# ucas-vg/PointTinyBenchmark

Measured on AMD Instinct MI355X. Metric: img/s (640x640) CPR R50-FPN fwd+loss, higher is better.
Workload: dtype fp32

## Files before the change

### include/cpr_hip.h

```cpp
#ifndef CPR_HIP_H
#define CPR_HIP_H
#ifdef __cplusplus
extern "C" {
#endif

#define CPR_ERR_ARG (-1001)
#define CPR_ERR_UNSUPPORTED (-1002)

int cpr_version(void);

#define CPR_CONV_RELU 1
#define CPR_CONV_OUT_BF16 2
#define CPR_CONV_RES_MASK 4
#define CPR_CONV_COLSUM 8
int cpr_conv2d_fwd(const float* in, const float* wgt, float* out, const float* scale, const float* bias,
                   const float* residual, const float* in_a, const float* in_b, float* gn_part, int N, int H, int W,
                   int Cin, int Cout, int KH, int KW, int stride, int pad, int Kpad, int flags, int in_relu,
                   int* variant_out, void* stream);

int cpr_conv2d_dual_fwd(const float* in, const float* wgt, const float* in2, const float* wgt2, float* out,
                        const float* scale, const float* bias, const float* scale2, const float* bias2, int N, int H, int W,
                        int Cin, int Cout, int KH, int KW, int stride, int pad, int Kpad, int H2, int W2, int Cin2,
                        int stride2, int Kpad2, int flags, int* variant_out, void* stream);

int cpr_conv1x1_stream_fwd(const float* in, const float* wgt, float* out, const float* scale, const float* bias,
                           const float* residual, long long M, int Cin, int Cout, int flags, void* stream);

int cpr_conv_wgrad_bf16_workspace(int N, int H, int W, int Cin, int Cout, int k);
int cpr_conv_wgrad_bf16(const void* dy, int dy_bf16, const void* x, int x_bf16, float* grad, void* ws, int N, int H, int W, int Cin,
                        int Cout, int k, int accumulate, void* stream);
int cpr_wgrad_bf16_set_tn(int on);
int cpr_conv_wgrad_bf16_workspace_s(int N, int H, int W, int Cin, int Cout, int k, int stride);
int cpr_conv_wgrad_bf16_s(const void* dy, int dy_bf16, const void* x, int x_bf16, float* grad, void* ws, int N, int H, int W, int Cin,
                          int Cout, int k, int stride, int accumulate, void* stream);

#define CPR_WINO_IN_B8 1
#define CPR_WINO_OUT_B8 2
int cpr_wino_pack_weights(const float* wgt, float* u, int Cin, int Cout, int Kpad, void* stream);
int cpr_conv3x3_wino_fwd(const float* in, const float* u, float* out, const float* scale, const float* bias,
                         const float* in_a, const float* in_b, float* gn_part, int N, int H, int W, int Cin, int Cout,
                         int flags, int in_relu, int layout, void* stream);
int cpr_wino32_pack_weights(const float* wgt, float* u, int Cin, int Cout, int Kpad, void* stream);
int cpr_conv3x3_wino32_slots(int H, int W);
int cpr_conv3x3_wino32_fwd(const float* in, const float* u, float* out, const float* scale, const float* bias,
                           const float* in_a, const float* in_b, float* gn_part, int N, int H, int W, int Cin, int Cout,
                           int flags, int in_relu, int layout, void* stream);
int cpr_gn_apply_b8(const float* x, const float* a, const float* b, float* y, int N, int H, int W, int C, int relu,
                    void* stream);

int cpr_conv2d_fwd_bf16(const void* in, const void* wgt, const void* wgt_frag, void* out, const float* scale, const float* bias,
                        const void* residual, float* gn_part, int N, int H, int W, int Cin, int Cout, int KH, int KW,
                        int stride, int pad, int Kpad, int relu, int out_fp32, int* variant_out, void* stream);
int cpr_conv2d_bf16_mask_slots(int N, int H, int W, int Cin, int Cout, int KH, int KW, int stride, int pad, int out_fp32);
int cpr_conv2d_dgrad_bf16_fused(const void* in, const void* wgt, const void* wgt_frag, float* out32, void* out16, const float* add32,
                                const void* mask, float* part, int N, int H, int W, int Cin, int Cout, int KH, int KW, int stride,
                                int pad, int Kpad, int* variant_out, void* stream);
int cpr_stem7x7s2_bf16(const float* in, const void* wgt, const float* scale, const float* bias, void* out, int N, int H, int W,
                       int relu, int layout, void* stream);
int cpr_stem7x7s2_pool_bf16(const float* in, const void* wgt, const float* scale, const float* bias, void* out, int N, int H,
                            int W, int layout, void* stream);
int cpr_maxpool3x3s2_bf16(const void* in, void* out, int N, int H, int W, int C, void* stream);
int cpr_gn_stats_bf16(const void* x, float* part, int N, int HW, int C, int P, void* stream);
int cpr_gn_apply_bf16(const void* x, const float* a, const float* b, const void* up, void* y, int N, int H, int W,
                      int C, int UH, int UW, int relu, void* stream);

int cpr_nchw_to_nhwc4(const float* in, float* out, int N, int C, int H, int W, void* stream);
int cpr_nhwc_to_nchw(const float* in, float* out, int N, int C, int H, int W, void* stream);
int cpr_stem7x7s2_pool_f32(const float* in, const float* wgt, const float* scale, const float* bias, float* out, int N, int H,
                           int W, int layout, void* stream);
// ... 177 lines not shown
int cpr_sgd_step(float* p, const float* grad, float* buf, const double* norm2, long long n, float lr, float mu, float wd,
                 float max_norm, float grad_scale, int first, void* stream);
int cpr_adam_step(float* p, const float* grad, float* exp_avg, float* exp_avg_sq, const double* norm2, long long n, double lr,
                  double beta1, double beta2, double eps, double wd, float step_size, float bc2_sqrt, float max_norm,
                  float grad_scale, int decoupled, void* stream);

int cpr_preprocess_u8(const unsigned char* img, const int* flip, const float* mean3, const float* stdinv3, int to_rgb,
                      float* out, int N, int H, int W, int Hp, int Wp, void* stream);
int cpr_clip_flip_boxes(float* boxes, const int* img_of, const int* flip, const int* img_hw, int n, int clip,
                        void* stream);

#ifdef CPR_BENCH_HOOKS
int cpr_conv_force_tile(int bm, int bn);
int cpr_conv_set_pipeline(int mode);
int cpr_conv_set_stream(int on);
int cpr_conv_set_ablation(int mode);
int cpr_wgrad_set_ablation(int mode);
int cpr_conv_set_extra_lds(int bytes);
int cpr_wino_set_variant(int sched, int ablate);
int cpr_bf16_set_dma(int on);
int cpr_bf16_set_wfrag(int on);
int cpr_wino_set_staging(int var, int tpx);
int cpr_wino32_set_debug(int ablate, int wg_per_cu, int stagger_pct);
int cpr_lsa_phase_clocks(long long* host_out, int reset);
#endif

#ifdef __cplusplus
}
#endif
#endif
```

### pointtinybenchmark_amd/_lib.py

```python
import ctypes
import os

_HERE = os.path.dirname(os.path.abspath(__file__))
LIB_PATH = os.path.join(_HERE, 'csrc', 'libcprhip.so')

_p = ctypes.c_void_p
_i = ctypes.c_int
_f = ctypes.c_float
_l = ctypes.c_longlong
_d = ctypes.c_double

SIGNATURES = {
    'cpr_version': [],
    'cpr_conv2d_fwd': [_p, _p, _p, _p, _p, _p, _p, _p, _p, _i, _i, _i, _i, _i, _i, _i, _i, _i, _i, _i, _i, _p, _p],
    'cpr_conv2d_dual_fwd': [_p] * 9 + [_i] * 16 + [_p, _p],
    'cpr_conv1x1_stream_fwd': [_p, _p, _p, _p, _p, _p, _l, _i, _i, _i, _p],
    'cpr_conv_wgrad_bf16_workspace': [_i, _i, _i, _i, _i, _i],
    'cpr_conv_wgrad_bf16_workspace_s': [_i] * 7,
    'cpr_conv_wgrad_bf16': [_p, _i, _p, _i, _p, _p, _i, _i, _i, _i, _i, _i, _i, _p],
    'cpr_conv_wgrad_bf16_s': [_p, _i, _p, _i, _p, _p] + [_i] * 8 + [_p],
    'cpr_wino_pack_weights': [_p, _p, _i, _i, _i, _p],
    'cpr_conv3x3_wino_fwd': [_p, _p, _p, _p, _p, _p, _p, _p, _i, _i, _i, _i, _i, _i, _i, _i, _p],
    'cpr_wino32_pack_weights': [_p, _p, _i, _i, _i, _p],
    'cpr_conv3x3_wino32_slots': [_i, _i],
    'cpr_conv3x3_wino32_fwd': [_p, _p, _p, _p, _p, _p, _p, _p, _i, _i, _i, _i, _i, _i, _i, _i, _p],
    'cpr_conv3x3_wino_wgrad_workspace': [_i, _i, _i, _i, _i],
    'cpr_conv3x3_wino_wgrad': [_p, _p, _p, _p, _p, _p, _i, _i, _i, _i, _i, _i, _i, _p],
    'cpr_gn_apply_b8': [_p, _p, _p, _p, _i, _i, _i, _i, _i, _p],
    'cpr_conv2d_fwd_bf16': [_p, _p, _p, _p, _p, _p, _p, _p] + [_i] * 12 + [_p, _p],
    'cpr_conv2d_bf16_mask_slots': [_i] * 10,
    'cpr_wgrad_bf16_set_tn': [_i],
    'cpr_bn_fold_multi': [_p, _i, _i, _p],
    'cpr_pack_weights_multi': [_p, _i, _i, _p],
    'cpr_pack_weights_bf16_multi': [_p, _i, _i, _p],
    'cpr_conv2d_dgrad_bf16_fused': [_p] * 8 + [_i] * 10 + [_p, _p],
    'cpr_stem7x7s2_bf16': [_p, _p, _p, _p, _p, _i, _i, _i, _i, _i, _p],
    'cpr_stem7x7s2_pool_bf16': [_p, _p, _p, _p, _p, _i, _i, _i, _i, _p],
    'cpr_maxpool3x3s2_bf16': [_p, _p, _i, _i, _i, _i, _p],
    'cpr_gn_stats_bf16': [_p, _p, _i, _i, _i, _i, _p],
    'cpr_gn_apply_bf16': [_p, _p, _p, _p, _p, _i, _i, _i, _i, _i, _i, _i, _p],
    'cpr_nchw_to_nhwc4': [_p, _p, _i, _i, _i, _i, _p],
    'cpr_nhwc_to_nchw': [_p, _p, _i, _i, _i, _i, _p],
    'cpr_stem7x7s2_pool_f32': [_p, _p, _p, _p, _p, _i, _i, _i, _i, _p],
    'cpr_maxpool3x3s2': [_p, _p, _i, _i, _i, _i, _p],
    'cpr_maxpool3x3s2_rec': [_p, _p, _p, _i, _i, _i, _i, _p],
    'cpr_maxpool3x3s2_bf16_rec': [_p, _p, _p, _i, _i, _i, _i, _p],
# ... 58 lines not shown
    'cpr_bn_apply': [_p] * 10 + [_l, _i, _i, _p],
    'cpr_bn_train_bwd': [_p] * 11 + [_l, _i, _p],
    'cpr_p2p_out_bf16_fwd': [_p] * 7 + [_i] * 5 + [_p],
    'cpr_p2p_out_bf16_dgrad': [_p, _i, _p, _p] + [_i] * 6 + [_p],
    'cpr_p2p_out_bf16_wgrad_ws': [_i] * 5,
    'cpr_p2p_out_bf16_wgrad': [_p] * 4 + [_i] + [_p] * 3 + [_i] * 5 + [_p],
    'cpr_p2p_loss_bwd': [_p] * 9 + [_i] * 5 + [_f] * 9 + [_p, _i, _i, _p],
    'cpr_p2p_loss_bwd_levels': [_p] * 7 + [_i] * 5 + [_p] * 6 + [_f] * 9 + [_p, _i, _i, _p],
    'cpr_grad_sumsq': [_p, _l, _p, _p, _i, _p],
    'cpr_sgd_step': [_p, _p, _p, _p, _l, _f, _f, _f, _f, _f, _i, _p],
    'cpr_adam_step': [_p, _p, _p, _p, _p, _l, _d, _d, _d, _d, _d, _f, _f, _f, _f, _i, _p],
}

BENCH_SIGNATURES = {
    'cpr_lsa_phase_clocks': [_p, _i],
    'cpr_wino32_set_debug': [_i, _i, _i],
    'cpr_conv_force_tile': [_i, _i],
    'cpr_conv_set_pipeline': [_i],
    'cpr_conv_set_stream': [_i],
    'cpr_conv_set_ablation': [_i],
    'cpr_wgrad_set_ablation': [_i],
    'cpr_wino_set_variant': [_i, _i],
    'cpr_wino_set_staging': [_i, _i],
    'cpr_conv_set_extra_lds': [_i],
    'cpr_bf16_set_dma': [_i],
    'cpr_bf16_set_wfrag': [_i],
}
BENCH_LIB_PATH = os.path.join(_HERE, 'csrc', 'libcprhip_bench.so')

_lib = None


class CprHipError(RuntimeError):
    pass


def load():
    global _lib
    if _lib is not None:
        return _lib
    path, sigs = LIB_PATH, dict(SIGNATURES)
    if os.environ.get('CPR_BENCH_HOOKS', '0') == '1':
        path = BENCH_LIB_PATH
        sigs.update(BENCH_SIGNATURES)
    if not os.path.exists(path):
        raise CprHipError('%s not found: run `python -m pointtinybenchmark_amd.build%s` (no CPU fallback exists)'
# ... 24 lines not shown
```

### pointtinybenchmark_amd/build.py

```python
import os
import subprocess
import sys

CSRC = os.path.join(os.path.dirname(os.path.abspath(__file__)), 'csrc')
LIB = os.path.join(CSRC, 'libcprhip.so')
SOURCES = ['conv_mfma.hip', 'conv1x1_stream.hip', 'conv_mfma_bf16.hip', 'conv_bf16_dma.hip', 'conv_bf16_pp.hip', 'stem_bf16.hip', 'stem_f32.hip', 'conv_wgrad_bf16.hip', 'conv_wgrad_bf16_tn.hip', 'conv_wgrad.hip', 'norm_pool.hip', 'cpr_points.hip', 'assign.hip',
           'postproc.hip', 'backward.hip', 'preprocess.hip', 'pack.hip', 'project.hip', 'conv_wino.hip', 'conv_wino32.hip', 'conv_wino_wgrad.hip', 'bn_train.hip',
           'p2p_out_bf16.hip', 'optim.hip', 'stem_bwd.hip']
HEADERS = ['common.h', 'conv_bf16_dma.h']
EXACT_SOURCES = {'cpr_points.hip', 'assign.hip', 'postproc.hip', 'preprocess.hip', 'optim.hip'}


def _hipcc():
    for c in (os.environ.get('HIPCC'), '/opt/rocm/bin/hipcc', 'hipcc'):
        if c and (os.path.isabs(c) and os.path.exists(c) or not os.path.isabs(c)):
            return c
    return 'hipcc'


def needs_build():
    if not os.path.exists(LIB):
        return True
    t = os.path.getmtime(LIB)
    deps = [os.path.join(CSRC, s) for s in SOURCES + HEADERS]
    return any(os.path.getmtime(d) > t for d in deps if os.path.exists(d))


BENCH_LIB = os.path.join(CSRC, 'libcprhip_bench.so')
HOOK_SOURCES = {'conv_mfma.hip', 'conv_wgrad.hip', 'conv_wino.hip', 'conv_mfma_bf16.hip', 'conv_bf16_dma.hip', 'conv_bf16_pp.hip', 'assign.hip', 'conv_wino32.hip'}


def build(force=False, verbose=True, bench_hooks=False):
    lib = BENCH_LIB if bench_hooks else LIB
    if not force and not (needs_build() if not bench_hooks else (
            not os.path.exists(lib) or any(os.path.getmtime(os.path.join(CSRC, s)) > os.path.getmtime(lib)
                                           for s in SOURCES + HEADERS))):
        return lib
    objs = []
    for s in SOURCES:
        src = os.path.join(CSRC, s)
        if not os.path.exists(src):
            continue
        hooked = bench_hooks and s in HOOK_SOURCES
        obj = os.path.join(CSRC, s.replace('.hip', '.bench.o' if hooked else '.o'))
        if bench_hooks and not hooked and os.path.exists(obj) and os.path.getmtime(obj) >= os.path.getmtime(src) \
                and all(os.path.getmtime(obj) >= os.path.getmtime(os.path.join(CSRC, h)) for h in HEADERS):
            objs.append(obj)
            continue
        cmd = [_hipcc(), '--offload-arch=gfx950', '-O3', '-std=c++17', '-fPIC'] + \
            (['-ffp-contract=off'] if s in EXACT_SOURCES else []) + (['-DCPR_BENCH_HOOKS'] if hooked else []) + \
            ['-c', src, '-o', obj]
        if verbose:
# ... 15 lines not shown
```

### pointtinybenchmark_amd/layers.py

```python
import os
import struct

import torch
import torch.nn as nn

from . import _lib, ops


_WEIGHT_EPOCH = [0]


def bump_weight_epoch():
    _WEIGHT_EPOCH[0] += 1


REFRESH_IN_PLACE = [os.environ.get('CPR_REFRESH_IN_PLACE', '1') != '0']

_FOLDS, _PACKS16, _PACKS32 = 'cpr_bn_fold_multi', 'cpr_pack_weights_bf16_multi', 'cpr_pack_weights_multi'


class FoldJob:
    multi = _FOLDS
    fold = None
    _ROW = struct.Struct('<7Qif')
# ... 13 lines not shown
    _ROW16, _ROW32 = struct.Struct('<4Q8i'), struct.Struct('<3Q10i')

    def __init__(self, weight, value, transpose, fold):
        self.weight, self.value, self.transpose, self.fold = weight, value, transpose, fold
        self.shape = O, I, KH, KW = weight.shape
        rows, cols = (I, O) if transpose else (O, I)
        bf16 = value.dtype == torch.bfloat16
        self.multi = _PACKS16 if bf16 else _PACKS32
        self.nblocks = max(1, min(64, (rows * (KH * KW * cols // 2 if bf16 else value.Kpad) + 255) // 256))

    def ptrs(self):
        pc = self.value
        return (self.weight.data_ptr(), 0 if self.fold is None else self.fold.value[0].data_ptr(), pc.w.data_ptr(),
                0 if pc.wfrag is None else pc.wfrag.data_ptr())

    def row(self, ptrs, block0):
        pc, nb = self.value, self.nblocks
        if self.multi is _PACKS16:
            return self._ROW16.pack(*ptrs, *self.shape, self.transpose, block0, nb, 0), block0 + nb
        return self._ROW32.pack(*ptrs[:3], nb, 0, *self.shape, pc.Cin, pc.Kpad, self.transpose, block0), block0 + nb

    def refresh_images(self, stream):
        pc = self.value
        for img, fn in ((pc.wino, 'cpr_wino_pack_weights'), (pc.wino32, 'cpr_wino32_pack_weights')):
            if img is not None:
                _lib.call(fn, pc.w.data_ptr(), img.data_ptr(), pc.Cin, pc.Cout, pc.Kpad, stream)


def _pack_job(pc, weight, transpose=0, fold=None):
    if isinstance(pc, ops.PackedConv) and weight.is_cuda and weight.dtype == torch.float32 and weight.is_contiguous() and \
            (pc.dtype == torch.float32 or ops.PACK_BF16_KERNEL[0]):
        return PackJob(weight, pc, transpose, fold)
    return None


class _Entry:
    __slots__ = ('tensors', 'ver', 'val', 'ready')

    def __init__(self, tensors, ver, val, ready):
        self.tensors, self.ver, self.val, self.ready = tensors, ver, val, ready


class _PackCache:

    def __init__(self):
        self._d = {}
        self._jobs = {}
# ... 177 lines not shown
```

### pointtinybenchmark_amd/ops.py

```python
import collections
import ctypes
import math
import os

import torch

from . import _lib


def _ptr(t):
    return ctypes.c_void_p(t.data_ptr()) if t is not None else None


def _stream():
    return ctypes.c_void_p(torch.cuda.current_stream().cuda_stream)


def _check(t, dtype=torch.float32):
    if not t.is_cuda:
        raise _lib.CprHipError('HIP op called with a CPU tensor: the product path has no CPU fallback')
    ok = t.dtype in dtype if isinstance(dtype, tuple) else t.dtype == dtype
    assert ok and t.is_contiguous(), (t.dtype, t.stride())
    return t

# ... 13 lines not shown


def nchw_to_nhwc(x):
    N, C, H, W = x.shape
    if C <= 4:
        x = _check(x.contiguous())
        out = torch.empty((N, H, W, 4), device=x.device, dtype=torch.float32)
        _lib.call('cpr_nchw_to_nhwc4', _ptr(x), _ptr(out), N, C, H, W, _stream())
        return out
    return x.permute(0, 2, 3, 1).contiguous()


def nhwc_to_nchw_dense(x_nhwc):
    N, H, W, C = x_nhwc.shape
    out = torch.empty((N, C, H, W), device=x_nhwc.device, dtype=torch.float32)
    _lib.call('cpr_nhwc_to_nchw', _ptr(_check(x_nhwc)), _ptr(out), N, C, H, W, _stream())
    return out


class PackedConv:
    wfrag = None
    wino = None
    wino32 = None
    ready = None

    def _packed(self):
        self.ready = record_ready()

    def __init__(self, weight, stride=1, padding=0, dtype=torch.float32):
        Cout, Cin, KH, KW = weight.shape
        w = weight.detach().to(torch.float32).permute(0, 2, 3, 1)
        self.dtype = dtype
        if dtype == torch.bfloat16:
            assert Cin % 64 == 0, 'bf16 conv needs Cin % 64 == 0'
            self.Cout, self.Cin, self.KH, self.KW, self.Kpad = Cout, Cin, KH, KW, KH * KW * Cin
            self.stride, self.padding = stride, padding
            if weight.is_cuda and PACK_BF16_KERNEL[0]:
                self._pack_bf16(weight, None, 0)
                return
            self.w = w.reshape(Cout, KH * KW * Cin).to(torch.bfloat16).contiguous()
            return
        if Cin <= 4:
            cin_p = 4
        else:
            assert Cin % 32 == 0, 'input channels must be a multiple of 32 (or <= 4 for the stem)'
            cin_p = Cin
# ... 100 lines not shown
    cur = torch.cuda.current_stream()
    if cur.cuda_stream != stream:
        cur.wait_event(ev)
    return ready


def pack_ready(pc):
    if pc.ready is not None:
        pc.ready = wait_ready(pc.ready)


def wino_eligible(pc, H, W, dtype=torch.float32):
    if not (WINOGRAD[0] and dtype == torch.float32 and pc.dtype == torch.float32 and pc.KH == 3 and pc.KW == 3 and
            pc.stride == 1 and pc.padding == 1 and pc.Cin % 16 == 0 and pc.Cin >= 32 and pc.Cout % 64 == 0):
        return False
    fill = (H * W) / float(((H + 15) // 16 * 16) * ((W + 15) // 16 * 16))
    return fill >= WINO_MIN_FILL


WINO_TILE = [os.environ.get('CPR_WINO_TILE', 'auto')]


def wino_instance(pc, H, W, fused_affine):
    can32 = pc.Cin % 8 == 0 and (not fused_affine or pc.Cin <= 256)
    if WINO_TILE[0] == '64' or not can32:
        return '64'
    if WINO_TILE[0] == '32':
        return '32'
    return WINO_AUTO(pc, H, W, fused_affine)


WINO32_MAX_PIXELS = 40 * 40


def WINO_AUTO(pc, H, W, fused_affine):
    return '32' if H * W <= WINO32_MAX_PIXELS else '64'


def wino_gn_slots(pc, H, W, fused_affine):
    if wino_instance(pc, H, W, fused_affine) == '32':
        return ((H + 7) // 8) * ((W + 15) // 16)
    return ((H + 15) // 16) * ((W + 15) // 16)


def is_b8(x):
    return x.dim() == 5 and x.shape[-1] == 8


def conv3x3_wino(x, pc, scale=None, bias=None, relu=False, gn_part=False, out=None, in_ab=None, in_relu=False,
                 out_b8=False):
    _check(x, ACT)
    in_b8 = is_b8(x)
    if in_b8:
        N, _, H, W, _ = x.shape
        Cin = x.shape[1] * 8
    else:
        N, H, W, Cin = x.shape
    assert x.dtype == torch.float32 and Cin == pc.Cin and pc.KH == 3 and pc.stride == 1 and pc.padding == 1
    inst = wino_instance(pc, H, W, in_ab is not None)
    attr, pack_fn = ('wino32', 'cpr_wino32_pack_weights') if inst == '32' else ('wino', 'cpr_wino_pack_weights')
    if getattr(pc, attr) is None:
        pack_ready(pc)
        wino = torch.empty((16 * pc.Cin * pc.Cout,), device=x.device, dtype=torch.float32)
        _lib.call(pack_fn, _ptr(pc.w), _ptr(wino), pc.Cin, pc.Cout, pc.Kpad, _stream())
        setattr(pc, attr, wino)
        pc._packed()
    pack_ready(pc)
    shape = (N, pc.Cout // 8, H, W, 8) if out_b8 else (N, H, W, pc.Cout)
    if out is None:
        out = torch.empty(shape, device=x.device, dtype=torch.float32)
    assert tuple(out.shape) == shape and out.is_contiguous()
    part = None
    if gn_part:
        part = torch.empty((N * wino_gn_slots(pc, H, W, in_ab is not None), pc.Cout, 2), device=x.device, dtype=torch.float32)
    a = b = None
    if in_ab is not None:
        a, b = in_ab
        assert Cin <= 512
    _lib.call('cpr_conv3x3_wino32_fwd' if inst == '32' else 'cpr_conv3x3_wino_fwd', _ptr(x), _ptr(getattr(pc, attr)), _ptr(out),
              _ptr(scale), _ptr(bias), _ptr(a), _ptr(b), _ptr(part), N, H, W, Cin, pc.Cout, CONV_RELU if relu else 0, int(in_relu),
              (1 if in_b8 else 0) | (2 if out_b8 else 0), _stream())
    if TRACE_CONV_VARIANT[0]:
        TRACE_CONV_VARIANT[1] = ('wino32' if inst == '32' else 'wino',
                                 (1 if in_b8 else 0) | (2 if out_b8 else 0) | (4 if in_ab is not None else 0))
    return (out, part) if gn_part else out


def gn_apply_b8(x, a=None, b=None, relu=False):
    assert is_b8(x)
    N, C8, H, W, _ = _check(x, ACT).shape
    y = torch.empty((N, H, W, C8 * 8), device=x.device, dtype=torch.float32)
    _lib.call('cpr_gn_apply_b8', _ptr(x), _ptr(a), _ptr(b), _ptr(y), N, H, W, C8 * 8, int(relu), _stream())
    return y


def conv2d(x, pc, scale=None, bias=None, residual=None, relu=False, in_ab=None, in_relu=False, gn_part=False,
           out=None, out_dtype=None, res_mask=False, colsum=False, out_b8=False):
    _check(x, ACT)
    pack_ready(pc)
    if is_b8(x):
        assert residual is None and not (res_mask or colsum) and out_dtype in (None, torch.float32) and \
            wino_eligible(pc, x.shape[2], x.shape[3], x.dtype), 'channel-blocked input needs a Winograd-eligible layer'
        return conv3x3_wino(x, pc, scale, bias, relu, gn_part, out, in_ab, in_relu, out_b8)
    N, H, W, Cin = x.shape
    assert Cin == pc.Cin, (Cin, pc.Cin)
    assert x.dtype == pc.dtype, 'weights were packed for %s, input is %s' % (pc.dtype, x.dtype)
    OH, OW = pc.out_hw(H, W)
# ... 1112 lines not shown
```

Baseline: 905.8.

## Add bf16 three-way-split Winograd 3x3 conv kernel for large wide layers

Adds a new Winograd F(2x2,3x3) forward kernel that splits fp32 transformed inputs and weights into three bf16 pieces (high, mid, low) and accumulates products with bf16 MFMA instructions, emulating fp32 accuracy. The auto-selector now routes 3x3 layers with at least 256 input and output channels and at least 160x160 pixels to this kernel, with a matching weight-packing path and weight-refresh hook. The aim is to replace slower fp32 matrix throughput with the higher bf16 MFMA rate on the largest FPN and head convolutions. The cost is several extra MFMAs per product, triple-size weight images, and a small residual precision difference from exact fp32.

```diff
diff --git a/include/cpr_hip.h b/include/cpr_hip.h
--- a/include/cpr_hip.h
+++ b/include/cpr_hip.h
@@ -45,6 +45,10 @@
 int cpr_conv3x3_wino32_fwd(const float* in, const float* u, float* out, const float* scale, const float* bias,
                            const float* in_a, const float* in_b, float* gn_part, int N, int H, int W, int Cin, int Cout,
                            int flags, int in_relu, int layout, void* stream);
+int cpr_wino_split_pack_weights(const float* wgt, void* u, int Cin, int Cout, int Kpad, void* stream);
+int cpr_conv3x3_wino_split_fwd(const float* in, const void* u, float* out, const float* scale, const float* bias,
+                               const float* in_a, const float* in_b, float* gn_part, int N, int H, int W, int Cin, int Cout,
+                               int flags, int in_relu, int layout, void* stream);
 int cpr_gn_apply_b8(const float* x, const float* a, const float* b, float* y, int N, int H, int W, int C, int relu,
                     void* stream);
 
@@ -268,6 +272,7 @@
 int cpr_bf16_set_wfrag(int on);
 int cpr_wino_set_staging(int var, int tpx);
 int cpr_wino32_set_debug(int ablate, int wg_per_cu, int stagger_pct);
+int cpr_wino_split_set_debug(int tpx, int scalar);
 int cpr_lsa_phase_clocks(long long* host_out, int reset);
 #endif
 
diff --git a/pointtinybenchmark_amd/_lib.py b/pointtinybenchmark_amd/_lib.py
--- a/pointtinybenchmark_amd/_lib.py
+++ b/pointtinybenchmark_amd/_lib.py
@@ -22,6 +22,8 @@
     'cpr_wino_pack_weights': [_p, _p, _i, _i, _i, _p],
     'cpr_conv3x3_wino_fwd': [_p, _p, _p, _p, _p, _p, _p, _p, _i, _i, _i, _i, _i, _i, _i, _i, _p],
     'cpr_wino32_pack_weights': [_p, _p, _i, _i, _i, _p],
+    'cpr_wino_split_pack_weights': [_p, _p, _i, _i, _i, _p],
+    'cpr_conv3x3_wino_split_fwd': [_p, _p, _p, _p, _p, _p, _p, _p, _i, _i, _i, _i, _i, _i, _i, _i, _p],
     'cpr_conv3x3_wino32_slots': [_i, _i],
     'cpr_conv3x3_wino32_fwd': [_p, _p, _p, _p, _p, _p, _p, _p, _i, _i, _i, _i, _i, _i, _i, _i, _p],
     'cpr_conv3x3_wino_wgrad_workspace': [_i, _i, _i, _i, _i],
@@ -126,6 +128,7 @@
     'cpr_wgrad_set_ablation': [_i],
     'cpr_wino_set_variant': [_i, _i],
     'cpr_wino_set_staging': [_i, _i],
+    'cpr_wino_split_set_debug': [_i, _i],
     'cpr_conv_set_extra_lds': [_i],
     'cpr_bf16_set_dma': [_i],
     'cpr_bf16_set_wfrag': [_i],
diff --git a/pointtinybenchmark_amd/build.py b/pointtinybenchmark_amd/build.py
--- a/pointtinybenchmark_amd/build.py
+++ b/pointtinybenchmark_amd/build.py
@@ -5,7 +5,7 @@
 CSRC = os.path.join(os.path.dirname(os.path.abspath(__file__)), 'csrc')
 LIB = os.path.join(CSRC, 'libcprhip.so')
 SOURCES = ['conv_mfma.hip', 'conv1x1_stream.hip', 'conv_mfma_bf16.hip', 'conv_bf16_dma.hip', 'conv_bf16_pp.hip', 'stem_bf16.hip', 'stem_f32.hip', 'conv_wgrad_bf16.hip', 'conv_wgrad_bf16_tn.hip', 'conv_wgrad.hip', 'norm_pool.hip', 'cpr_points.hip', 'assign.hip',
-           'postproc.hip', 'backward.hip', 'preprocess.hip', 'pack.hip', 'project.hip', 'conv_wino.hip', 'conv_wino32.hip', 'conv_wino_wgrad.hip', 'bn_train.hip',
+           'postproc.hip', 'backward.hip', 'preprocess.hip', 'pack.hip', 'project.hip', 'conv_wino.hip', 'conv_wino32.hip', 'conv_wino_split.hip', 'conv_wino_wgrad.hip', 'bn_train.hip',
            'p2p_out_bf16.hip', 'optim.hip', 'stem_bwd.hip']
 HEADERS = ['common.h', 'conv_bf16_dma.h']
 EXACT_SOURCES = {'cpr_points.hip', 'assign.hip', 'postproc.hip', 'preprocess.hip', 'optim.hip'}
@@ -27,7 +27,7 @@
 
 
 BENCH_LIB = os.path.join(CSRC, 'libcprhip_bench.so')
-HOOK_SOURCES = {'conv_mfma.hip', 'conv_wgrad.hip', 'conv_wino.hip', 'conv_mfma_bf16.hip', 'conv_bf16_dma.hip', 'conv_bf16_pp.hip', 'assign.hip', 'conv_wino32.hip'}
+HOOK_SOURCES = {'conv_mfma.hip', 'conv_wgrad.hip', 'conv_wino.hip', 'conv_mfma_bf16.hip', 'conv_bf16_dma.hip', 'conv_bf16_pp.hip', 'assign.hip', 'conv_wino32.hip', 'conv_wino_split.hip'}
 
 
 def build(force=False, verbose=True, bench_hooks=False):
diff --git a/pointtinybenchmark_amd/csrc/conv_wino_split.hip b/pointtinybenchmark_amd/csrc/conv_wino_split.hip
--- /dev/null
+++ b/pointtinybenchmark_amd/csrc/conv_wino_split.hip
@@ -0,0 +1,533 @@
+#include "common.h"
+
+typedef __bf16 bf16x8 __attribute__((ext_vector_type(8)));
+typedef __bf16 bf16x4 __attribute__((ext_vector_type(4)));
+typedef __bf16 bf16x2 __attribute__((ext_vector_type(2)));
+typedef float f32x2 __attribute__((ext_vector_type(2)));
+typedef unsigned u32x4 __attribute__((ext_vector_type(4)));
+
+struct WinoSplitParams {
+    const float* in;
+    const __bf16* u;
+    float* out;
+    const float* scale;
+    const float* bias;
+    float* gn_part;
+    const float* in_a;
+    const float* in_b;
+    int in_relu, out_b8;
+    int N, H, W, Cin, Cout, relu, RY, RX, regions, tilesN, nch;
+    int tpx;
+};
+
+constexpr int SPLIT_UCHUNK = 16 * 2 * 3 * 256;
+constexpr int SPLIT_VBUF = 3 * 16 * 64 * 8;
+
+__device__ __forceinline__ void split3(f32x2 x, bf16x2& h, bf16x2& m, bf16x2& l) {
+    h = __builtin_convertvector(x, bf16x2);
+    const f32x2 r = x - __builtin_convertvector(h, f32x2);
+    m = __builtin_convertvector(r, bf16x2);
+    const f32x2 s = r - __builtin_convertvector(m, f32x2);
+    l = __builtin_convertvector(s, bf16x2);
+}
+
+__device__ __forceinline__ float sadd(float a, float b) { float r; asm("v_add_f32 %0, %1, %2" : "=v"(r) : "v"(a), "v"(b)); return r; }
+__device__ __forceinline__ float ssub(float a, float b) { float r; asm("v_sub_f32 %0, %1, %2" : "=v"(r) : "v"(a), "v"(b)); return r; }
+__device__ __forceinline__ float sfma(float a, float b, float c) {
+    float r; asm("v_fma_f32 %0, %1, %2, %3" : "=v"(r) : "v"(a), "v"(b), "v"(c)); return r;
+}
+__device__ __forceinline__ void split3s(float x0, float x1, bf16x2& h, bf16x2& m, bf16x2& l) {
+    h = __builtin_convertvector(f32x2{x0, x1}, bf16x2);
+    const float r0 = ssub(x0, (float)h[0]), r1 = ssub(x1, (float)h[1]);
+    m = __builtin_convertvector(f32x2{r0, r1}, bf16x2);
+    l = __builtin_convertvector(f32x2{ssub(r0, (float)m[0]), ssub(r1, (float)m[1])}, bf16x2);
+}
+
+__global__ void wino_split_pack_kernel(const float* __restrict__ w, __bf16* __restrict__ u, int Cin, int Cout, int Kpad) {
+    const int idx = blockIdx.x * blockDim.x + threadIdx.x;
+    if (idx >= Cin * Cout) return;
+    const int ci = idx % Cin, co = idx / Cin;
+    float g[3][3];
+#pragma unroll
+    for (int a = 0; a < 3; ++a)
+#pragma unroll
+        for (int b = 0; b < 3; ++b) g[a][b] = w[(size_t)co * Kpad + (a * 3 + b) * Cin + ci];
+    float t[4][3];
+#pragma unroll
+    for (int b = 0; b < 3; ++b) {
+        t[0][b] = g[0][b];
+        t[1][b] = 0.5f * (g[0][b] + g[1][b] + g[2][b]);
+        t[2][b] = 0.5f * (g[0][b] - g[1][b] + g[2][b]);
+        t[3][b] = g[2][b];
+    }
+    const int tn = co >> 6, cl = co & 63, chunk = ci >> 3, k = ci & 7, nch = Cin >> 3;
+    __bf16* dst = u + (size_t)(tn * nch + chunk) * SPLIT_UCHUNK + (cl >> 5) * 3 * 256 + (cl & 31) * 8 + k;
+#pragma unroll
+    for (int i = 0; i < 4; ++i) {
+        const float v[4] = {t[i][0], 0.5f * (t[i][0] + t[i][1] + t[i][2]), 0.5f * (t[i][0] - t[i][1] + t[i][2]), t[i][2]};
+#pragma unroll
+        for (int j = 0; j < 4; j += 2) {
+            bf16x2 h, m, l;
+            split3(f32x2{v[j], v[j + 1]}, h, m, l);
+#pragma unroll
+            for (int e = 0; e < 2; ++e) {
+                __bf16* d = dst + (i * 4 + j + e) * (2 * 3 * 256);
+                d[0] = h[e]; d[256] = m[e]; d[512] = l[e];
+            }
+        }
+    }
+}
+
+template <bool INB8, bool XF, bool SC>
+__global__ __launch_bounds__(512, 1) void conv_wino_split_kernel(WinoSplitParams p) {
+    constexpr int XFMAX = 512;
+    constexpr int RAWROW = 148;
+    constexpr int RAWBUF = 18 * RAWROW;
+    constexpr int VFLOATS = SPLIT_VBUF;
+    constexpr int KLOOP = VFLOATS + 2 * RAWBUF;
+    constexpr int EPI = 8 * 64 * 64;
+    constexpr int BASE = KLOOP > EPI ? KLOOP : EPI;
+    __shared__ __attribute__((aligned(16))) float smem[BASE + (XF ? 4 * XFMAX : 0)];
+    __bf16* Vs = reinterpret_cast<__bf16*>(smem);
+    float* Rw = smem + VFLOATS;
+    float* ABs = smem + BASE;
+
+    const int tid = threadIdx.x, lane = tid & 63;
+    const int wave = __builtin_amdgcn_readfirstlane(tid >> 6);
+    const int l31 = lane & 31, half = lane >> 5;
+
+    const int pixbytes = INB8 ? 32 : p.Cin * 4;
+    const int chunk_bytes = INB8 ? p.H * p.W * 32 : 32;
+    const __amdgpu_buffer_rsrc_t rs_in = __builtin_amdgcn_make_buffer_rsrc(
+        const_cast<float*>(p.in), 0, (int)((size_t)p.N * p.H * p.W * p.Cin * 4), 0x00020000);
+    const __amdgpu_buffer_rsrc_t rs_u = __builtin_amdgcn_make_buffer_rsrc(
+        const_cast<__bf16*>(p.u), 0, (int)((size_t)p.tilesN * p.nch * SPLIT_UCHUNK * 2), 0x00020000);
+    int par = 0;
+    int upyx[2], raw_wr[2];
+#pragma unroll
+    for (int k = 0; k < 2; ++k) {
+        const int pix = (tid + 512 * k) >> 1;
+        const int py = pix / 18, px = pix - py * 18;
+        upyx[k] = py << 8 | px;
+        raw_wr[k] = py * RAWROW + px * 8 + (tid & 1) * 4;
+    }
+    const bool second_unit = wave < 3;
+    const bool unit1_live = tid + 512 < 648;
+    const int ti = wave >> 1, ttl = (tid >> 1) & 63, tch = tid & 1;
+    const int t_ra = ti == 0 ? 0 : ti == 2 ? 2 : 1;
+    const int t_rb = ti == 0 ? 2 : ti == 1 ? 2 : ti == 2 ? 1 : 3;
+    const float t_sg = ti == 1 ? 1.f : -1.f;
+    const float* t_rd = Rw + (2 * (ttl & 7)) * RAWROW + (2 * (ttl >> 3)) * 8 + 4 * tch;
+    __bf16* const t_wr = Vs + (ti * 4) * 512 + ttl * 8 + 4 * tch;
+    const int last = p.nch - 1;
+    const float relu_floor = (XF && p.in_relu) ? 0.f : -INFINITY;
+
+    struct Tile {
+        int rg, tn, n, oy0, ox0, n0;
+        int voffA[2];
+        unsigned uok;
+        bool any_pad, valid;
+    };
+    const int T = p.regions * p.tilesN;
+    const int per = (T + 7) >> 3;
+    const int ngrp = p.tpx > 0 ? p.tilesN / p.tpx : 1;
+    const int per_r = p.tpx > 0 ? (p.regions * ngrp + 7) / 8 : 0;
+    auto setup = [&](int vb) {
+        Tile t;
+        if (p.tpx > 0) {
+            const int x = vb & 7, s = vb >> 3;
+            const int sr = s / p.tpx;
+            t.rg = (x / ngrp) * per_r + sr;
+            t.tn = (x % ngrp) * p.tpx + (s - sr * p.tpx);
+            t.valid = sr < per_r && t.rg < p.regions;
+            if (!t.valid) { t.rg = 0; t.tn = 0; }
+        } else {
+            const int tile = (vb & 7) * per + (vb >> 3);
+            t.valid = vb < per * 8 && tile < T;
+            const int tl = t.valid ? tile : 0;
+            t.rg = tl / p.tilesN; t.tn = tl - t.rg * p.tilesN;
+        }
+        t.n = t.rg / (p.RY * p.RX);
+        const int rrem = t.rg - t.n * p.RY * p.RX;
+        const int ry = rrem / p.RX, rx = rrem - ry * p.RX;
+        t.oy0 = ry * 16; t.ox0 = rx * 16; t.n0 = t.tn * 64;
+        const int img_base = INB8 ? (t.n * (p.Cin >> 3)) * p.H * p.W * 32 : t.n * p.H * p.W * p.Cin * 4;
+        t.uok = 0;
+#pragma unroll
+        for (int k = 0; k < 2; ++k) {
+            const int iy = t.oy0 - 1 + (upyx[k] >> 8), ix = t.ox0 - 1 + (upyx[k] & 255);
+            const bool ok = (k == 0 || unit1_live) & ((unsigned)iy < (unsigned)p.H) & ((unsigned)ix < (unsigned)p.W);
+            t.uok |= (ok ? 1u : 0u) << k;
+            t.voffA[k] = ok ? img_base + (iy * p.W + ix) * pixbytes + (tid & 1) * 16 : (int)0x80000000;
+        }
+        t.any_pad = XF && __builtin_amdgcn_ballot_w64(t.uok != (unit1_live ? 3u : 1u)) != 0;
+        return t;
+    };
+
+    f32x4 sp[2][2];
+    bf16x8 bx[2][2], by[2][2];
+    float tab_a = 0.f, tab_b = 0.f;
+    Tile cur = setup(blockIdx.x);
+    auto ld_a = [&](const Tile& t, int ck, int k) {
+        return __builtin_bit_cast(f32x4, __builtin_amdgcn_raw_buffer_load_b128(rs_in, t.voffA[k], ck * chunk_bytes, 0));
+    };
+    const int ub_x = (half ? 1 : 0) * 512 + l31 * 16, ub_y = (half ? 2 : 0) * 512 + l31 * 16;
+    auto ld_u = [&](int tn, int ck, int fl, int nb) {
+        const int f = 2 * wave + fl;
+        const int soff = (tn * p.nch + ck) * (SPLIT_UCHUNK * 2) + (f * 2 + nb) * 3 * 512;
+        bx[fl][nb] = __builtin_bit_cast(bf16x8, __builtin_amdgcn_raw_buffer_load_b128(rs_u, ub_x, soff, 0));
+        by[fl][nb] = __builtin_bit_cast(bf16x8, __builtin_amdgcn_raw_buffer_load_b128(rs_u, ub_y, soff, 0));
+    };
+    auto prefetch = [&](const Tile& t) {
+        sp[0][0] = ld_a(t, 0, 0); sp[1][0] = ld_a(t, 1, 0);
+        if (second_unit) { sp[0][1] = ld_a(t, 0, 1); sp[1][1] = ld_a(t, 1, 1); }
+#pragma unroll
+        for (int fl = 0; fl < 2; ++fl)
+#pragma unroll
+            for (int nb = 0; nb < 2; ++nb) ld_u(t.tn, 0, fl, nb);
+        if (XF) {
+            if (tid < p.Cin) { tab_a = p.in_a[t.n * p.Cin + tid]; tab_b = p.in_b[t.n * p.Cin + tid]; }
+        }
+    };
+    auto affine = [&](f32x4 v, f32x4 a4, f32x4 b4, int k) {
+        if (SC) v = f32x4{sfma(v.x, a4.x, b4.x), sfma(v.y, a4.y, b4.y), sfma(v.z, a4.z, b4.z), sfma(v.w, a4.w, b4.w)};
+        else v = v * a4 + b4;
+        v.x = fmaxf(v.x, relu_floor); v.y = fmaxf(v.y, relu_floor); v.z = fmaxf(v.z, relu_floor); v.w = fmaxf(v.w, relu_floor);
+        if (cur.any_pad) {
+            asm volatile("");
+            if (!((cur.uok >> k) & 1u)) v = f32x4{0.f, 0.f, 0.f, 0.f};
+        }
+        return v;
+    };
+    auto r_a = [&](f32x4 v, int chunk, int buf, int k) {
+        if (k == 1 && !second_unit) return;
+        if (XF) {
+            const float* tab = ABs + par * 2 * XFMAX + (chunk < last ? chunk : last) * 8 + (tid & 1) * 4;
+            v = affine(v, *reinterpret_cast<const f32x4*>(tab), *reinterpret_cast<const f32x4*>(tab + XFMAX), k);
+        }
+        if (k == 0 || unit1_live) *reinterpret_cast<f32x4*>(Rw + buf * RAWBUF + raw_wr[k]) = v;
+    };
+    f32x4 tr[4], ta[4];
+    auto t_read = [&](int buf, int s0) {
+#pragma unroll
+        for (int s = 0; s < 2; ++s) {
+            ta[2 * s] = *reinterpret_cast<const f32x4*>(t_rd + buf * RAWBUF + t_ra * RAWROW + (s0 + s) * 8);
+            ta[2 * s + 1] = *reinterpret_cast<const f32x4*>(t_rd + buf * RAWBUF + t_rb * RAWROW + (s0 + s) * 8);
+        }
+    };
+    auto t_pass = [&](int s0) {
+#pragma unroll
+        for (int s = 0; s < 2; ++s) {
+            const f32x4 a = ta[2 * s], b = ta[2 * s + 1];
+            if (SC) tr[s0 + s] = f32x4{sfma(t_sg, b.x, a.x), sfma(t_sg, b.y, a.y), sfma(t_sg, b.z, a.z), sfma(t_sg, b.w, a.w)};
+            else tr[s0 + s] = a + t_sg * b;
+        }
+    };
+    auto t_col = [&](int buf, int j) {
+        bf16x2 h0, m0, l0, h1, m1, l1;
+        if (SC) {
+            const f32x4 a = j == 0 ? tr[0] : j == 1 ? tr[1] : j == 2 ? tr[2] : tr[1];
+            const f32x4 b = j == 0 ? tr[2] : j == 1 ? tr[2] : j == 2 ? tr[1] : tr[3];
+            float o[4];
+#pragma unroll
+            for (int e = 0; e < 4; ++e) o[e] = j == 1 ? sadd(a[e], b[e]) : ssub(a[e], b[e]);
+            split3s(o[0], o[1], h0, m0, l0);
+            split3s(o[2], o[3], h1, m1, l1);
+        } else {
+            const f32x4 o = j == 0 ? tr[0] - tr[2] : j == 1 ? tr[1] + tr[2] : j == 2 ? tr[2] - tr[1] : tr[1] - tr[3];
+            split3(f32x2{o.x, o.y}, h0, m0, l0);
+            split3(f32x2{o.z, o.w}, h1, m1, l1);
+        }
+        __bf16* d = t_wr + buf * SPLIT_VBUF + j * 512;
+        *reinterpret_cast<bf16x4*>(d) = bf16x4{h0.x, h0.y, h1.x, h1.y};
+        *reinterpret_cast<bf16x4*>(d + 16 * 512) = bf16x4{m0.x, m0.y, m1.x, m1.y};
+        *reinterpret_cast<bf16x4*>(d + 32 * 512) = bf16x4{l0.x, l0.y, l1.x, l1.y};
+    };
+    const __bf16* a_lds = Vs + (2 * wave) * 512 + l31 * 8;
+    const int a3_plane = half ? 0 : 2;
+    bf16x8 fa[3];
+    auto a_read = [&](int buf, int fl, int tb, int z) {
+        const __bf16* b0 = a_lds + buf * SPLIT_VBUF + fl * 512 + tb * 256;
+        fa[z] = *reinterpret_cast<const bf16x8*>(b0 + (z == 0 ? 0 : z == 1 ? 16 * 512 : a3_plane * 16 * 512));
+    };
+
+    if (cur.valid) prefetch(cur);
+    if (XF) {
+        if (tid < p.Cin) { ABs[tid] = tab_a; ABs[XFMAX + tid] = tab_b; }
+        __syncthreads();
+    }
+    for (int vb = blockIdx.x; cur.valid; vb += gridDim.x) {
+    const int rg = cur.rg, n = cur.n, oy0 = cur.oy0, ox0 = cur.ox0, n0 = cur.n0;
+
+    f32x16 acc[2][2][2];
+#pragma unroll
+    for (int fl = 0; fl < 2; ++fl)
+#pragma unroll
+        for (int tb = 0; tb < 2; ++tb)
+#pragma unroll
+            for (int nb = 0; nb < 2; ++nb)
+#pragma unroll
+                for (int r = 0; r < 16; ++r) acc[fl][tb][nb][r] = 0.f;
+
+    r_a(sp[0][0], 0, 0, 0); r_a(sp[0][1], 0, 0, 1);
+    r_a(sp[1][0], 1, 1, 0); r_a(sp[1][1], 1, 1, 1);
+    sp[0][0] = ld_a(cur, 2 < last ? 2 : last, 0);
+    if (second_unit) sp[0][1] = ld_a(cur, 2 < last ? 2 : last, 1);
+    __syncthreads();
+    t_read(0, 0); t_pass(0); t_read(0, 2); t_pass(2);
+#pragma unroll
+    for (int j = 0; j < 4; ++j) t_col(0, j);
+    __syncthreads();
+#pragma unroll
+    for (int z = 0; z < 3; ++z) a_read(0, 0, 0, z);
+
+#define SMFMA(FL, TB)                                                                                            \
+    do {                                                                                                         \
+        acc[FL][TB][0] = __builtin_amdgcn_mfma_f32_32x32x16_bf16(fa[0], bx[FL][0], acc[FL][TB][0], 0, 0, 0);   \
+        q_fill(q++);                                                                                             \
+        acc[FL][TB][1] = __builtin_amdgcn_mfma_f32_32x32x16_bf16(fa[0], bx[FL][1], acc[FL][TB][1], 0, 0, 0);   \
+        q_fill(q++);                                                                                             \
+        acc[FL][TB][0] = __builtin_amdgcn_mfma_f32_32x32x16_bf16(fa[1], bx[FL][0], acc[FL][TB][0], 0, 0, 0);   \
+        q_fill(q++);                                                                                             \
+        acc[FL][TB][1] = __builtin_amdgcn_mfma_f32_32x32x16_bf16(fa[1], bx[FL][1], acc[FL][TB][1], 0, 0, 0);   \
+        q_fill(q++);                                                                                             \
+        acc[FL][TB][0] = __builtin_amdgcn_mfma_f32_32x32x16_bf16(fa[2], by[FL][0], acc[FL][TB][0], 0, 0, 0);   \
+        q_fill(q++);                                                                                             \
+        acc[FL][TB][1] = __builtin_amdgcn_mfma_f32_32x32x16_bf16(fa[2], by[FL][1], acc[FL][TB][1], 0, 0, 0);   \
+        q_fill(q++);                                                                                             \
+    } while (0)
+    for (int c = 0; c < p.nch; ++c) {
+        const int buf = c & 1, nbuf = buf ^ 1;
+        const int cn = c + 1 < last ? c + 1 : last;
+        auto q_fill = [&](int q) {
+            if (q & 1) {
+                const int g = q / 6 + 1, z = (q % 6) >> 1;
+                if (g < 4) a_read(buf, g >> 1, g & 1, z);
+                else a_read(nbuf, 0, 0, z);
+            }
+            switch (q) {
+                case 0: t_read(nbuf, 0); break;
+                case 2: t_pass(0); t_read(nbuf, 2); break;
+                case 3: t_pass(2); break;
+                case 4: t_col(nbuf, 0); break;
+                case 6: t_col(nbuf, 1); break;
+                case 8: t_col(nbuf, 2); break;
+                case 10: t_col(nbuf, 3); break;
+                case 12: ld_u(cur.tn, cn, 0, 0); ld_u(cur.tn, cn, 0, 1); break;
+                case 13: r_a(sp[0][0], c + 2, buf, 0); break;
+                case 14: r_a(sp[0][1], c + 2, buf, 1); break;
+                case 17:
+                    asm volatile("" ::: "memory");
+                    __builtin_amdgcn_s_waitcnt(0xc07f);
+                    __builtin_amdgcn_s_barrier();
+                    asm volatile("" ::: "memory");
+                    break;
+                case 18: {
+                    const int c3 = c + 3 < last ? c + 3 : last;
+                    sp[0][0] = ld_a(cur, c3, 0);
+                    if (second_unit) sp[0][1] = ld_a(cur, c3, 1);
+                    break;
+                }
+                case 23: ld_u(cur.tn, cn, 1, 0); ld_u(cur.tn, cn, 1, 1); break;
+                default: break;
+            }
+            __builtin_amdgcn_sched_barrier(0);
+        };
+        int q = 0;
+        SMFMA(0, 0);
+        SMFMA(0, 1);
+        SMFMA(1, 0);
+        SMFMA(1, 1);
+    }
+#undef SMFMA
+
+    const Tile nxt = setup(vb + gridDim.x);
+    if (nxt.valid) prefetch(nxt);
+    __syncthreads();
+    float* Rs = smem;
+    const int ei = wave >> 1, ejp = wave & 1;
+    if (ejp) {
+#pragma unroll
+        for (int tb = 0; tb < 2; ++tb)
+#pragma unroll
+            for (int nb = 0; nb < 2; ++nb)
+#pragma unroll
+                for (int r = 0; r < 16; ++r) {
+                    const int trow = tb * 32 + (r & 3) + 8 * (r >> 2) + 4 * half;
+                    const float m2 = acc[0][tb][nb][r], m3 = acc[1][tb][nb][r];
+                    Rs[((ei * 2 + 0) * 64 + trow) * 64 + nb * 32 + l31] = m2;
+                    Rs[((ei * 2 + 1) * 64 + trow) * 64 + nb * 32 + l31] = -m2 - m3;
+                }
+    }
+    __syncthreads();
+    if (!ejp) {
+#pragma unroll
+        for (int tb = 0; tb < 2; ++tb)
+#pragma unroll
+            for (int nb = 0; nb < 2; ++nb)
+#pragma unroll
+                for (int r = 0; r < 16; ++r) {
+                    const int trow = tb * 32 + (r & 3) + 8 * (r >> 2) + 4 * half;
+                    const float m0 = acc[0][tb][nb][r], m1 = acc[1][tb][nb][r];
+                    float* r0 = Rs + ((ei * 2 + 0) * 64 + trow) * 64 + nb * 32 + l31;
+                    float* r1 = Rs + ((ei * 2 + 1) * 64 + trow) * 64 + nb * 32 + l31;
+                    *r0 = (m0 + m1) + *r0;
+                    *r1 = m1 + *r1;
+                }
+    }
+    __syncthreads();
+    const int c4 = tid & 15;
+    const int co = n0 + c4 * 4;
+    f32x4 sc = {1.f, 1.f, 1.f, 1.f}, bi = {0.f, 0.f, 0.f, 0.f};
+    if (p.scale) sc = *reinterpret_cast<const f32x4*>(p.scale + co);
+    if (p.bias) bi = *reinterpret_cast<const f32x4*>(p.bias + co);
+    const __amdgpu_buffer_rsrc_t rs_out = __builtin_amdgcn_make_buffer_rsrc(
+        p.out, 0, (int)((size_t)p.N * p.H * p.W * p.Cout * 4), 0x00020000);
+    f32x4 gs = {0.f, 0.f, 0.f, 0.f}, gq = {0.f, 0.f, 0.f, 0.f};
+#pragma unroll
+    for (int k = 0; k < 2; ++k) {
+        const int t = (tid >> 4) + 32 * k;
+        const int oy = oy0 + 2 * (t & 7), ox = ox0 + 2 * (t >> 3);
+#pragma unroll
+        for (int b = 0; b < 2; ++b) {
+            const f32x4 r0 = *reinterpret_cast<const f32x4*>(Rs + ((0 * 2 + b) * 64 + t) * 64 + c4 * 4);
+            const f32x4 r1 = *reinterpret_cast<const f32x4*>(Rs + ((1 * 2 + b) * 64 + t) * 64 + c4 * 4);
+            const f32x4 r2 = *reinterpret_cast<const f32x4*>(Rs + ((2 * 2 + b) * 64 + t) * 64 + c4 * 4);
+            const f32x4 r3 = *reinterpret_cast<const f32x4*>(Rs + ((3 * 2 + b) * 64 + t) * 64 + c4 * 4);
+            f32x4 y[2] = {r0 + r1 + r2, r1 - r2 - r3};
+#pragma unroll
+            for (int a = 0; a < 2; ++a) {
+                f32x4 v = y[a] * sc + bi;
+                if (p.relu) { v.x = fmaxf(v.x, 0.f); v.y = fmaxf(v.y, 0.f); v.z = fmaxf(v.z, 0.f); v.w = fmaxf(v.w, 0.f); }
+                const bool ok = (oy + a < p.H) & (ox + b < p.W);
+                const unsigned off = !ok ? 0x80000000u
+                    : p.out_b8 ? (unsigned)((((n * (p.Cout >> 3) + (co >> 3)) * p.H + oy + a) * p.W + ox + b) * 8 + (co & 7)) * 4u
+                               : (unsigned)(((n * p.H + oy + a) * p.W + ox + b) * p.Cout + co) * 4u;
+                __builtin_amdgcn_raw_buffer_store_b128(__builtin_bit_cast(u32x4, v), rs_out, (int)off, 0, 0);
+                if (p.gn_part && ok) { gs += v; gq += v * v; }
+            }
+        }
+    }
+    if (p.gn_part) {
+#pragma unroll
+        for (int e = 0; e < 4; ++e) {
+            gs[e] += __shfl_xor(gs[e], 16, 64); gs[e] += __shfl_xor(gs[e], 32, 64);
+            gq[e] += __shfl_xor(gq[e], 16, 64); gq[e] += __shfl_xor(gq[e], 32, 64);
+        }
+        __syncthreads();
+        if (lane < 16) {
+#pragma unroll
+            for (int e = 0; e < 4; ++e) {
+                smem[(wave * 64 + c4 * 4 + e) * 2 + 0] = gs[e];
+                smem[(wave * 64 + c4 * 4 + e) * 2 + 1] = gq[e];
+            }
+        }
+        __syncthreads();
+        if (tid < 64) {
+            float s = 0.f, q = 0.f;
+#pragma unroll
+            for (int w8 = 0; w8 < 8; ++w8) { s += smem[(w8 * 64 + tid) * 2]; q += smem[(w8 * 64 + tid) * 2 + 1]; }
+            float* dst = p.gn_part + ((size_t)rg * p.Cout + n0 + tid) * 2;
+            dst[0] = s; dst[1] = q;
+        }
+    }
+    if (XF && tid < p.Cin) {
+        ABs[(par ^ 1) * 2 * XFMAX + tid] = tab_a;
+        ABs[(par ^ 1) * 2 * XFMAX + XFMAX + tid] = tab_b;
+    }
+    par ^= 1;
+    __syncthreads();
+    cur = nxt;
+    }
+}
+
+#ifdef CPR_BENCH_HOOKS
+static int split_tpx = -1, split_scalar = -1;
+extern "C" int cpr_wino_split_set_debug(int tpx, int scalar) {
+    CPR_CHECK_ARG(tpx >= -1 && tpx <= 2 && scalar >= -1 && scalar <= 1);
+    split_tpx = tpx;
+    split_scalar = scalar;
+    return CPR_OK;
+}
+#else
+constexpr int split_tpx = -1, split_scalar = -1;
+#endif
+constexpr int SPLIT_TPX_DEFAULT = 0, SPLIT_SCALAR_DEFAULT = 0;
+
+extern "C" int cpr_wino_split_pack_weights(const float* wgt, void* u, int Cin, int Cout, int Kpad, hipStream_t stream) {
+    CPR_CHECK_ARG(wgt && u && Cin > 0 && Cout > 0 && Cin % 8 == 0 && Cout % 64 == 0 && Kpad >= 9 * Cin);
+    hipLaunchKernelGGL(wino_split_pack_kernel, dim3(cdiv(Cin * Cout, 256)), dim3(256), 0, stream, wgt,
+                       static_cast<__bf16*>(u), Cin, Cout, Kpad);
+    CPR_LAUNCH_STATUS();
+}
+
+static int wino_split_launch(const float* in, const void* u, float* out, const float* scale, const float* bias,
+                             const float* in_a, const float* in_b, float* gn_part, int N, int H, int W, int Cin,
+                             int Cout, int flags, int in_relu, int layout, hipStream_t stream) {
+    CPR_CHECK_ARG(in && u && out && N > 0 && H > 0 && W > 0);
+    CPR_CHECK_ARG(Cin > 0 && Cout > 0 && Cin % 16 == 0 && Cout % 64 == 0 && Cin >= 32);
+    CPR_CHECK_ARG((flags & ~CPR_CONV_RELU) == 0 && (layout & ~3) == 0);
+    if (in_a) CPR_CHECK_ARG(in_b && Cin <= 512);
+    if ((long long)N * H * W * Cin * 4 >= (1ll << 31) || (long long)N * H * W * Cout * 4 >= (1ll << 31)) return CPR_ERR_UNSUPPORTED;
+    if ((long long)Cin * Cout * 96 >= (1ll << 31)) return CPR_ERR_UNSUPPORTED;
+    WinoSplitParams p;
+    p.in = in; p.u = static_cast<const __bf16*>(u); p.out = out; p.scale = scale; p.bias = bias; p.gn_part = gn_part;
+    p.in_a = in_a; p.in_b = in_b; p.in_relu = in_relu; p.out_b8 = (layout & CPR_WINO_OUT_B8) ? 1 : 0;
+    p.N = N; p.H = H; p.W = W; p.Cin = Cin; p.Cout = Cout; p.relu = flags & CPR_CONV_RELU;
+    p.RY = (H + 15) / 16; p.RX = (W + 15) / 16;
+    p.regions = N * p.RY * p.RX; p.tilesN = Cout / 64; p.nch = Cin / 8;
+    const long long T = (long long)p.regions * p.tilesN;
+    if (T >= (1ll << 30)) return CPR_ERR_UNSUPPORTED;
+    static int cu_of_device[64] = {};
+    int dev = 0, ncu = 256;
+    if (hipGetDevice(&dev) == hipSuccess && dev >= 0 && dev < 64) {
+        if (cu_of_device[dev] == 0) {
+            int v = 0;
+            if (hipDeviceGetAttribute(&v, hipDeviceAttributeMultiprocessorCount, dev) == hipSuccess && v > 0) cu_of_device[dev] = v;
+        }
+        if (cu_of_device[dev] > 0) ncu = cu_of_device[dev];
+    }
+    ncu = (ncu + 7) / 8 * 8;
+    int grid = (int)((T + 7) / 8 * 8);
+    if (grid > ncu) grid = ncu;
+    p.tpx = split_tpx >= 0 ? split_tpx : SPLIT_TPX_DEFAULT;
+    if (p.tpx > 0 && !(p.tilesN % p.tpx == 0 && 8 % (p.tilesN / p.tpx) == 0)) p.tpx = 0;
+    if (p.tpx > 0) {
+        const long long per_r = ((long long)p.regions * (p.tilesN / p.tpx) + 7) / 8;
+        const long long vbs = 8 * per_r * p.tpx;
+        if (vbs < grid) grid = (int)vbs;
+    }
+    const bool b8 = (layout & CPR_WINO_IN_B8) != 0, xf = in_a != nullptr;
+    const bool sc = (split_scalar >= 0 ? split_scalar : SPLIT_SCALAR_DEFAULT) != 0;
+#define SLAUNCH(SC_)                                                                                                         \
+    do {                                                                                                                     \
+        if (b8 && xf) hipLaunchKernelGGL((conv_wino_split_kernel<true, true, SC_>), dim3(grid), dim3(512), 0, stream, p);    \
+        else if (b8) hipLaunchKernelGGL((conv_wino_split_kernel<true, false, SC_>), dim3(grid), dim3(512), 0, stream, p);    \
+        else if (xf) hipLaunchKernelGGL((conv_wino_split_kernel<false, true, SC_>), dim3(grid), dim3(512), 0, stream, p);    \
+        else hipLaunchKernelGGL((conv_wino_split_kernel<false, false, SC_>), dim3(grid), dim3(512), 0, stream, p);           \
+    } while (0)
+#ifdef CPR_BENCH_HOOKS
+    if (sc != (SPLIT_SCALAR_DEFAULT != 0)) { if (sc) SLAUNCH(true); else SLAUNCH(false); } else
+#endif
+    SLAUNCH(SPLIT_SCALAR_DEFAULT != 0);
+#undef SLAUNCH
+    CPR_LAUNCH_STATUS();
+}
+
+extern "C" int cpr_conv3x3_wino_split_fwd(const float* in, const void* u, float* out, const float* scale, const float* bias,
+                                          const float* in_a, const float* in_b, float* gn_part, int N, int H, int W, int Cin,
+                                          int Cout, int flags, int in_relu, int layout, hipStream_t stream) {
+    CPR_CHECK_ARG(N > 0 && H > 0 && W > 0 && Cin > 0 && Cout > 0);
+    const int per = cpr_images_per_launch(N, (long long)H * W * cpr_max2(Cin, Cout) * 4);
+    if (per <= 0) return CPR_ERR_UNSUPPORTED;
+    const size_t slots = (size_t)((H + 15) / 16) * ((W + 15) / 16);
+    for (int n0 = 0; n0 < N; n0 += per) {
+        const int n = N - n0 < per ? N - n0 : per;
+        const int rc = wino_split_launch(in + (size_t)n0 * H * W * Cin, u, out + (size_t)n0 * H * W * Cout, scale, bias,
+                                         in_a ? in_a + (size_t)n0 * Cin : nullptr, in_b ? in_b + (size_t)n0 * Cin : nullptr,
+                                         gn_part ? gn_part + (size_t)n0 * slots * Cout * 2 : nullptr, n, H, W, Cin, Cout, flags,
+                                         in_relu, layout, stream);
+        if (rc != CPR_OK) return rc;
+    }
+    return CPR_OK;
+}
diff --git a/pointtinybenchmark_amd/layers.py b/pointtinybenchmark_amd/layers.py
--- a/pointtinybenchmark_amd/layers.py
+++ b/pointtinybenchmark_amd/layers.py
@@ -59,7 +59,8 @@
 
     def refresh_images(self, stream):
         pc = self.value
-        for img, fn in ((pc.wino, 'cpr_wino_pack_weights'), (pc.wino32, 'cpr_wino32_pack_weights')):
+        for img, fn in ((pc.wino, 'cpr_wino_pack_weights'), (pc.wino32, 'cpr_wino32_pack_weights'),
+                        (pc.wino_split, 'cpr_wino_split_pack_weights')):
             if img is not None:
                 _lib.call(fn, pc.w.data_ptr(), img.data_ptr(), pc.Cin, pc.Cout, pc.Kpad, stream)
 
diff --git a/pointtinybenchmark_amd/ops.py b/pointtinybenchmark_amd/ops.py
--- a/pointtinybenchmark_amd/ops.py
+++ b/pointtinybenchmark_amd/ops.py
@@ -59,6 +59,7 @@
     wfrag = None
     wino = None
     wino32 = None
+    wino_split = None
     ready = None
 
     def _packed(self):
@@ -205,6 +206,8 @@
 
 
 def wino_instance(pc, H, W, fused_affine):
+    if WINO_TILE[0] == 'split':
+        return 'split'
     can32 = pc.Cin % 8 == 0 and (not fused_affine or pc.Cin <= 256)
     if WINO_TILE[0] == '64' or not can32:
         return '64'
@@ -214,16 +217,26 @@
 
 
 WINO32_MAX_PIXELS = 40 * 40
+WINO_SPLIT_MIN_PIXELS = 160 * 160
 
 
 def WINO_AUTO(pc, H, W, fused_affine):
-    return '32' if H * W <= WINO32_MAX_PIXELS else '64'
+    if H * W <= WINO32_MAX_PIXELS:
+        return '32'
+    if pc.Cin >= 256 and pc.Cout >= 256 and H * W >= WINO_SPLIT_MIN_PIXELS:
+        return 'split'
+    return '64'
 
 
 def wino_gn_slots(pc, H, W, fused_affine):
     if wino_instance(pc, H, W, fused_affine) == '32':
         return ((H + 7) // 8) * ((W + 15) // 16)
     return ((H + 15) // 16) * ((W + 15) // 16)
+
+
+WINO_IMAGES = {'64': ('wino', 'cpr_wino_pack_weights', 16, torch.float32, 'cpr_conv3x3_wino_fwd'),
+               '32': ('wino32', 'cpr_wino32_pack_weights', 16, torch.float32, 'cpr_conv3x3_wino32_fwd'),
+               'split': ('wino_split', 'cpr_wino_split_pack_weights', 48, torch.bfloat16, 'cpr_conv3x3_wino_split_fwd')}
 
 
 def is_b8(x):
@@ -241,10 +254,10 @@
         N, H, W, Cin = x.shape
     assert x.dtype == torch.float32 and Cin == pc.Cin and pc.KH == 3 and pc.stride == 1 and pc.padding == 1
     inst = wino_instance(pc, H, W, in_ab is not None)
-    attr, pack_fn = ('wino32', 'cpr_wino32_pack_weights') if inst == '32' else ('wino', 'cpr_wino_pack_weights')
+    attr, pack_fn, per_w, img_dtype, fwd_fn = WINO_IMAGES[inst]
     if getattr(pc, attr) is None:
         pack_ready(pc)
-        wino = torch.empty((16 * pc.Cin * pc.Cout,), device=x.device, dtype=torch.float32)
+        wino = torch.empty((per_w * pc.Cin * pc.Cout,), device=x.device, dtype=img_dtype)
         _lib.call(pack_fn, _ptr(pc.w), _ptr(wino), pc.Cin, pc.Cout, pc.Kpad, _stream())
         setattr(pc, attr, wino)
         pc._packed()
@@ -260,12 +273,12 @@
     if in_ab is not None:
         a, b = in_ab
         assert Cin <= 512
-    _lib.call('cpr_conv3x3_wino32_fwd' if inst == '32' else 'cpr_conv3x3_wino_fwd', _ptr(x), _ptr(getattr(pc, attr)), _ptr(out),
+    _lib.call(fwd_fn, _ptr(x), _ptr(getattr(pc, attr)), _ptr(out),
               _ptr(scale), _ptr(bias), _ptr(a), _ptr(b), _ptr(part), N, H, W, Cin, pc.Cout, CONV_RELU if relu else 0, int(in_relu),
               (1 if in_b8 else 0) | (2 if out_b8 else 0), _stream())
     if TRACE_CONV_VARIANT[0]:
-        TRACE_CONV_VARIANT[1] = ('wino32' if inst == '32' else 'wino',
-                                 (1 if in_b8 else 0) | (2 if out_b8 else 0) | (4 if in_ab is not None else 0))
+        TRACE_CONV_VARIANT[1] = ('bf16', 0) if inst == 'split' else (
+            'wino32' if inst == '32' else 'wino', (1 if in_b8 else 0) | (2 if out_b8 else 0) | (4 if in_ab is not None else 0))
     return (out, part) if gn_part else out
 
 
```

Result: faster. 975.7 (median of 6 runs) (+7.7%).
